# Vasilispapg/CVML-GoalNet

Measured on AMD Instinct MI355X. Metric: training clips/sec at batch 64, 16-frame 224² clips; logit MAE vs CPU ref, higher is better.
Workload: dtype f32; 1 GPU; AVM train step (forward + broadcast-MSE + backward + fused Adam), 64 clips x 16 frames = 1024 frames of 3x224x224 + 30x30 MFCC per GPU; dropout live (device masks), BatchNorm train mode; frames_per_gpu=1024, h=224, w=224, parallelism=dp1, ddp_semantics=local BN + local MSE per rank, gradient mean (standard DDP), params=1286754369

## Files before the change

### __graft_entry__.py

```python
from __future__ import annotations

import glob
import os
import subprocess
import sys

ROOT = os.path.dirname(os.path.abspath(__file__))
PKG = os.path.join(ROOT, "cvml_goalnet_amd")
CSRC = os.path.join(PKG, "csrc")
LIB = os.path.join(PKG, "libgoalnet_hip.so")
HIPCC = os.environ.get("HIPCC", "/opt/rocm/bin/hipcc")
FLAGS = ["--offload-arch=gfx950", "-O3", "-std=c++17", "-fPIC", "-Wall", "-Wno-unused-function"]


def _stale(target, sources):
    if not os.path.exists(target):
        return True
    t = os.path.getmtime(target)
    return any(os.path.getmtime(s) > t for s in sources)


def build(force: bool = False) -> None:
    srcs = sorted(glob.glob(os.path.join(CSRC, "*.hip")))
    hdrs = sorted(glob.glob(os.path.join(CSRC, "*.h"))) + [os.path.join(ROOT, "include", h) for h in ("goalnet_hip.h", "goalnet_loss.h")]
    objdir = os.path.join(CSRC, "build")
    os.makedirs(objdir, exist_ok=True)
    objs = []
    procs = []
    for s in srcs:
        o = os.path.join(objdir, os.path.basename(s)[:-4] + ".o")
        objs.append(o)
        if force or _stale(o, [s] + hdrs):
            procs.append((s, subprocess.Popen([HIPCC, *FLAGS, "-c", s, "-o", o])))
    for s, p in procs:
        if p.wait() != 0:
            raise RuntimeError(f"hipcc failed on {s}")
    if force or procs or _stale(LIB, objs):
        subprocess.check_call([HIPCC, "--offload-arch=gfx950", "-shared", "-fPIC", "-o", LIB, *objs])
    if ROOT not in sys.path:
        sys.path.insert(0, ROOT)
    import cvml_goalnet_amd
    from cvml_goalnet_amd import _lib
    lib = _lib.load()
    assert lib.goalnet_abi_version() == _lib.ABI_VERSION


def smoke() -> None:
    if ROOT not in sys.path:
        sys.path.insert(0, ROOT)
    import numpy as np
    import torch
    from cvml_goalnet_amd import AVM, synth
    from oracle import avm_ref

    assert torch.cuda.is_available(), "smoke() needs the GPU"
    torch.cuda.set_device(0)
    n, h = 4, 40
    params = synth.make_params(h, h)
    vis = torch.from_numpy(synth.make_visual(n, h, h))
    aud = torch.from_numpy(synth.make_audio(n))
    lab = torch.from_numpy(synth.make_labels(n))
    masks = [torch.from_numpy(m) for m in synth.make_drop_masks(n)]

    model = AVM(audio_included=True, device="cuda:0", seed=synth.BASE_SEED)
    sd = {k: torch.from_numpy(v) for k, v in params.items()}
    sd.update(avm_ref.init_buffers())
    model.load_state_dict(sd)
    loss, pred = model.train_step(aud.cuda(), vis.cuda(), lab.cuda())
    torch.cuda.synchronize()

    p = {k: torch.from_numpy(v.copy()) for k, v in params.items()}
    o_loss, o_pred, o_g = avm_ref.train_step(p, avm_ref.init_buffers(), {}, aud, vis, lab, masks, True)
    err = (pred.cpu() - o_pred.view(-1)).abs().max().item()
    lerr = abs(loss.item() - o_loss.item())
    new = model.state_dict()
    gerr = perr = 0.0
    for k, og in o_g.items():
# ... 16 lines not shown
```

### cvml_goalnet_amd/_lib.py

```python
from __future__ import annotations

import ctypes
import os
from ctypes import c_char_p, c_double, c_float, c_int, c_int64, c_size_t, c_uint32, c_uint64, c_void_p

_HERE = os.path.dirname(os.path.abspath(__file__))
LIB_PATH = os.environ.get("GOALNET_LIB_PATH") or os.path.join(_HERE, "libgoalnet_hip.so")
ABI_VERSION = 7
STAT_PARTS = 1024
ADAM_RANGES_MAX = 32

P = c_void_p


class RowCopy(ctypes.Structure):
    _fields_ = [("src", c_void_p), ("dst", c_void_p), ("row_bytes", c_int64), ("nrows", c_int), ("gather", c_int), ("cursor", c_void_p),
                ("cursor_bias", c_int64)]


class AdamRange(ctypes.Structure):
    _fields_ = [("begin", c_int64), ("count", c_int64), ("skipped", c_int64)]


PROTOTYPES = {
# ... 91 lines not shown
    "goalnet_mse_bcast": (c_int, [P, P, c_int, P, P, P]),
    "goalnet_cubic_resample": (c_int, [P, P, P, c_int64, c_int, c_int, P]),
    "goalnet_logmel_slots": (c_int, [P, P, P, c_int, c_int, P, P, P, P, P, P, P, P]),
    "goalnet_mfcc_from_logmel": (c_int, [P, P, c_int, c_int, P, P, P, P, c_int, c_int, c_double, P]),
    "goalnet_cls_head_fwd": (c_int, [P, c_int64, P, P, P, P, c_int, c_int, c_int, P]),
    "goalnet_cross_entropy": (c_int, [P, P, P, P, c_int, c_int, P]),
    "goalnet_cls_head_bwd": (c_int, [P, P, P, c_int64, P, P, c_int64, P, c_int64, P, P, c_int, c_int, c_int, P]),
    "goalnet_argmax_plus1": (c_int, [P, P, c_int, c_int, P]),
    "goalnet_adam_step": (c_int, [P, P, P, P, c_int64, c_double, c_double, c_double, c_double, c_int, c_float, P]),
    "goalnet_counter_add": (c_int, [P, c_int64, P]),
    "goalnet_dropout_masks_dev": (c_int, [P, c_int, ctypes.POINTER(c_int), c_int, c_uint64, c_uint32, c_uint32, P, c_float, c_int64, P]),
    "goalnet_adam_step_dev": (c_int, [P, P, P, P, c_int64, c_double, c_double, c_double, c_double, P, c_int64, c_float, P]),
    "goalnet_adam_step_dev_blocks": (c_int, [P, P, P, P, c_int64, c_double, c_double, c_double, c_double, P, c_int64, c_float, c_int, P]),
    "goalnet_adam_step_dev_shadow": (c_int, [P, P, P, P, c_int64, c_double, c_double, c_double, c_double, P, c_int64, c_float, P, c_int64,
                                             c_int64, c_int, P]),
    "goalnet_adam_step_dev_guarded": (c_int, [P, P, P, P, c_int64, c_double, c_double, c_double, c_double, P, c_int64, c_float, P, c_int64,
                                              c_int64, c_int, P, P]),
    "goalnet_adam_step_dev_ranges": (c_int, [P, P, P, P, ctypes.POINTER(AdamRange), c_int, c_double, c_double, c_double, c_double, P, c_float,
                                             P, c_int64, c_int64, c_int, P, P]),
    "goalnet_scale": (c_int, [P, c_int64, c_float, P]),
    "goalnet_grad_finite_check": (c_int, [P, c_int64, P, c_int64, P, P, P]),
    "goalnet_counters_add4": (c_int, [P, c_int64, c_int64, c_int64, c_int64, P]),
    "goalnet_counters_add4_guarded": (c_int, [P, c_int64, c_int64, c_int64, c_int64, P, P]),
    "goalnet_rows_scatter_tick": (c_int, [ctypes.POINTER(RowCopy), c_int, P, c_int64, c_int64, c_int64, c_int64, P, P]),
    "goalnet_rows_copy_batch": (c_int, [ctypes.POINTER(RowCopy), c_int, P]),
    "goalnet_frames_preprocess": (c_int, [P, c_int, c_int, c_int, P, c_int, c_int, P, P]),
    "goalnet_frames_preprocess_strided": (c_int, [P, c_int, c_int, c_int, c_int, P, c_int, c_int, P, P]),
    "goalnet_gather_clips_ws_bytes": (c_size_t, [c_int]),
    "goalnet_gather_clips": (c_int, [P, c_int, c_int64, P, P, c_int, P, c_int64, P, P, P, P, c_size_t, P]),
    "goalnet_kts_ws_bytes": (c_size_t, [c_int, c_int, c_int]),
    "goalnet_kts": (c_int, [P, c_int, c_int, c_int, c_int, c_int, c_int, c_double, c_int, c_int, P, P, P, P, P, P, P, c_size_t, P]),
    "goalnet_rank_corr": (c_int, [P, c_int64, c_int, P, c_int64, c_int, c_int, c_int, c_int, P, P, P, P, P, P, P]),
    "goalnet_knapsack_ws_bytes": (c_size_t, [c_int, c_int]),
    "goalnet_knapsack": (c_int, [P, P, c_int, c_int, P, P, c_size_t, P]),
    "goalnet_fscore": (c_int, [P, P, c_int, c_int, P, P, P]),
    "goalnet_postprocess_ws_bytes": (c_size_t, [c_int, c_int, c_int]),
    "goalnet_postprocess": (c_int, [P, c_int, c_int, c_int, P, c_int, c_int, c_int, P, c_int, P, P, P, P, P, P, P, c_size_t, P]),
    "goalnet_postprocess_batch_ws_bytes": (c_size_t, [c_int, c_int, c_int, c_int]),
    "goalnet_postprocess_batch": (c_int, [P, c_int, c_int, c_int, c_int, P, c_int, c_int, c_int, P, c_int, P, P, P, P, P, P, P, c_size_t, P]),
    "goalnet_postprocess_batch_kernel_name": (c_char_p, [c_int, c_int]),
    "goalnet_mean_annotations": (c_int, [P, c_int, c_int, c_int, P, P, P]),
    "goalnet_rows_gather": (c_int, [P, P, c_int64, c_int, P, P]),
    "goalnet_rows_scatter": (c_int, [P, P, c_int64, c_int, P, P]),
}

LOSS_PROTOTYPES = {
    "goalnet_frame_loss_ws_bytes": (c_size_t, [c_int, c_int]),
    "goalnet_frame_loss": (c_int, [c_int, c_double, P, P, P, c_int, P, P, P, c_size_t, P]),
    "goalnet_mlp_fwd_loss": (c_int, [P, c_int64, c_int, P, P, P, P, P, P, P, P, P, P, P, c_int, c_double, P, c_int, P, P]),
}
LOSS_KINDS = {"mse_bcast": 0, "mse": 1, "l1": 2, "smooth_l1": 3, "rank": 4}
FRAME_LOSS_MAX_N = 65536

_lib = None


class GoalnetError(RuntimeError):
    pass


def load():
    global _lib
    if _lib is not None:
        return _lib
    if not os.path.exists(LIB_PATH):
        raise GoalnetError(
            f"{LIB_PATH} not found: build it with `python -c 'import __graft_entry__ as g; g.build()'`. "
            "There is no CPU / eager fallback for the AVM hot path.")
    lib = ctypes.CDLL(LIB_PATH)
    for name, (res, args) in (*PROTOTYPES.items(), *LOSS_PROTOTYPES.items()):
        fn = getattr(lib, name)
        fn.restype = res
        fn.argtypes = args
    v = lib.goalnet_abi_version()
    if v != ABI_VERSION:
        raise GoalnetError(f"libgoalnet_hip.so ABI {v} != expected {ABI_VERSION}")
    _lib = lib
    return lib


def check(rc: int, what: str = ""):
    if rc != 0:
        msg = load().goalnet_last_error()
        raise GoalnetError(f"{what}: rc={rc}: {msg.decode() if msg else ''}")
```

### cvml_goalnet_amd/csrc/gemm_f32.hip

```cpp
#include <stdlib.h>

#include "adam.h"
#include "gemm_common.h"
#include "skinny.h"

using namespace goalnet;

namespace {

constexpr int BM = 128, BN = 128, BK = 32;
constexpr int LDR = 128;
constexpr int OP_FLOATS = BM * BK;

__device__ __forceinline__ int kc_off(int row, int chunk) { return row * BK + ((chunk ^ ((row >> 1) & 7)) << 2); }

__device__ __forceinline__ float4 f4zero() { return make_float4(0.f, 0.f, 0.f, 0.f); }
__device__ __forceinline__ float4 f4fma(float4 v, float4 s, float4 t) {
    return make_float4(fmaf(v.x, s.x, t.x), fmaf(v.y, s.y, t.y), fmaf(v.z, s.z, t.z), fmaf(v.w, s.w, t.w));
}

typedef unsigned int u32x4 __attribute__((ext_vector_type(4)));
constexpr unsigned OOB = 0xFFFFFF00u;

__device__ __forceinline__ float4 f4sel(bool v, float4 a) { return v ? a : f4zero(); }

__device__ __forceinline__ __amdgpu_buffer_rsrc_t make_rsrc(const void* base, uint32_t bytes) {
    return __builtin_amdgcn_make_buffer_rsrc(const_cast<void*>(base), 0, (int)bytes, 0x00020000);
}
__device__ __forceinline__ float4 bload(__amdgpu_buffer_rsrc_t r, unsigned voff, unsigned soff) {
    const u32x4 v = __builtin_amdgcn_raw_buffer_load_b128(r, (int)voff, (int)soff, 0);
    return make_float4(__uint_as_float(v.x), __uint_as_float(v.y), __uint_as_float(v.z), __uint_as_float(v.w));
}
__device__ __forceinline__ uint32_t clamp_u32(int64_t v) {
    return v <= 0 ? 0u : (v > 0xFFFFFF00ll ? 0xFFFFFF00u : (uint32_t)v);
}

template <bool AFFINE>
struct KCLoader {
    struct P {
        const float* x; int64_t ld; int rows;
        const float* scale; const float* shift; int bnC;
        int convC;
    };
    static constexpr bool KC = true;
    static constexpr bool STRIP = false;
    static constexpr bool ONE_STAGE = false;
    static constexpr int ONE_STAGE_BLOCKS = 3;
    __amdgpu_buffer_rsrc_t rx, rsc, rsh;
    unsigned voff[4], vaff;
    int bnC, convC;
    float4 sc, sh;
    __device__ KCLoader(const P& p, int row0, int tid) {
        const int nrows = p.rows - row0 < BM ? p.rows - row0 : BM;
        rx = make_rsrc(p.x + (int64_t)row0 * p.ld, clamp_u32((int64_t)nrows * p.ld * 4));
// ... 896 lines not shown
            a.x = fmaf(-shv.x, u, a.x); a.y = fmaf(-shv.y, u, a.y); a.z = fmaf(-shv.z, u, a.z); a.w = fmaf(-shv.w, u, a.w);
        }
        if (ok && g == 0) {
            float* o = ep.out + row * ep.ld + col;
            o[0] = epi_apply(ep, a.x, row, col);
            o[1] = epi_apply(ep, a.y, row, col + 1);
            o[2] = epi_apply(ep, a.z, row, col + 2);
            o[3] = epi_apply(ep, a.w, row, col + 3);
        }
    }
}

constexpr bool EPI_PAIR_DX = true;
static int epi_store_mode(const EpiP& ep, bool a_kc, bool b_kc) {
    const char* e = getenv("GOALNET_F32_EPI_STORE");
    if ((e && e[0] == '0') || !a_kc) return EPI_ST_GLOBAL;
    const bool slab = ep.slab_stride > 0;
    const int mode = slab ? EPI_RAW : ep.mode;
    const int64_t ld = (slab && ep.slabs) ? (int64_t)ep.cols : ep.ld;
    if (mode != EPI_RAW && mode != EPI_BIAS_RELU) return EPI_ST_GLOBAL;
    if (ep.rows <= 0 || ep.cols <= 0 || ld < ep.cols || (int64_t)BM * ld * 4 >= 0xFFFFFF00ll) return EPI_ST_GLOBAL;
    if (e && e[0] == '1') return EPI_ST_BUF;
    return (EPI_PAIR_DX && !b_kc && mode == EPI_RAW) ? EPI_ST_BUF_PAIR : EPI_ST_BUF;
}

template <class AL, class BL, bool N64 = false>
int launch_gemm(const char* name, const typename AL::P& ap, const typename BL::P& bp, const EpiP& ep,
                int64_t M, int64_t N, int ktiles, int nsplit, int m_fast, hipStream_t st) {
    const int64_t tiles_m = (M + BM - 1) / BM, tiles_n = (N + (N64 ? 64 : BN) - 1) / (N64 ? 64 : BN);
    GN_REQUIRE(tiles_m * tiles_n < (1ll << 31), GOALNET_E_SHAPE, "%s: too many tiles", name);
    GN_REQUIRE(nsplit >= 1 && nsplit <= 65535, GOALNET_E_SHAPE, "%s: bad split count %d", name, nsplit);
    const int kps = (ktiles + nsplit - 1) / nsplit;
    GN_REQUIRE(!ep.tile_ctr || (ktiles + kps - 1) / kps == nsplit, GOALNET_E_SHAPE, "%s: fused split-K needs every split non-empty", name);
    const bool xcd_local = nsplit >= 8 && tiles_m * tiles_n <= 256 && tiles_m * tiles_n * ((nsplit + 7) / 8 * 8) < (1ll << 31);
    dim3 grid((unsigned)(tiles_m * tiles_n), (unsigned)nsplit, 1);
    if (xcd_local) grid = dim3((unsigned)(tiles_m * tiles_n * ((nsplit + 7) / 8 * 8)), 1, 1);
    static const int force_stages = getenv("GOALNET_F32_STAGES") ? atoi(getenv("GOALNET_F32_STAGES")) : 0;
    const int epi_st = epi_store_mode(ep, AL::KC, BL::KC);
    const bool one_stage = AL::STRIP || force_stages == 1 || (force_stages != 2 && AL::ONE_STAGE);
    if (one_stage) {
        hipLaunchKernelGGL((gemm_f32_kernel<AL, BL, N64, 1>), grid, dim3(256), 0, st, ap, bp, ep, (int)tiles_m, (int)tiles_n,
                           (m_fast & 1) | (epi_st << 1), ktiles, kps, xcd_local ? nsplit : 0);
        GN_LAUNCH_CHECK(name);
        return 0;
    }
    if constexpr (!AL::STRIP) {
        hipLaunchKernelGGL((gemm_f32_kernel<AL, BL, N64>), grid, dim3(256), 0, st, ap, bp, ep, (int)tiles_m, (int)tiles_n,
                           (m_fast & 1) | (epi_st << 1), ktiles, kps, xcd_local ? nsplit : 0);
        GN_LAUNCH_CHECK(name);
    }
    return 0;
}

}

namespace goalnet {
int launch_splitk_reduce(const char* name, const float* slabs, int nsplit, int64_t slab_stride, const EpiP& ep, hipStream_t st) {
    const int64_t total = (int64_t)ep.rows * (ep.cols >> 2);
    int64_t blocks = (total + 255) / 256;
    if (blocks > 4096) blocks = 4096;
    if (blocks < 1) blocks = 1;
    if (total < 65536 && nsplit >= 32) {
        int64_t wb = (total + 15) / 16;
        if (wb > 4096) wb = 4096;
        hipLaunchKernelGGL(splitk_reduce_wide_kernel, dim3((unsigned)wb), dim3(256), 0, st, slabs, nsplit, slab_stride, ep);
        GN_LAUNCH_CHECK(name);
        return 0;
    }
    hipLaunchKernelGGL(splitk_reduce_kernel, dim3((unsigned)blocks), dim3(256), 0, st, slabs, nsplit, slab_stride, ep);
    GN_LAUNCH_CHECK(name);
    return 0;
}

int pick_splits(int64_t tiles, int ktiles) {
    if (ktiles < 8 || (ktiles < 64 && tiles >= 128)) return 1;
    int64_t s = ((ktiles < 64 ? 256 : 1024) + tiles - 1) / tiles;
    const int64_t smax = ktiles < 64 ? ktiles / 4 : (ktiles / 8 > 1 ? ktiles / 8 : 1);
    if (s > smax) s = smax;
    if (s < 1) s = 1;
    const int kps = (int)((ktiles + s - 1) / s);
    return (ktiles + kps - 1) / kps;
}

}

extern "C" {

static int conv_splits_f32(int64_t M, int Cin, int Cout) {
    return conv_fwd_splits(((M + BM - 1) / BM) * ((Cout + BN - 1) / BN), 9 * Cin / BK);
}

constexpr bool CONV_STRIP_FWD = true;
constexpr bool CONV_STRIP_DGRAD = true;
static bool conv_strip_f32(int W, int nsplit, bool narrow, bool affine) {
    const char* e = getenv("GOALNET_F32_CONV_STRIP");
    if (e && e[0] == '0') return false;
    return nsplit == 1 && !narrow && W <= CONV_STRIP_MAX_W && (affine ? CONV_STRIP_FWD : CONV_STRIP_DGRAD);
}

size_t goalnet_conv3x3_fwd_ws_bytes(int N, int H, int W, int Cin, int Cout) {
    if (N <= 0 || H <= 0 || W <= 0 || Cin <= 0 || Cout <= 0) return 0;
    const int64_t M = (int64_t)N * H * W;
    const int s = conv_splits_f32(M, Cin, Cout);
    return s > 1 ? (size_t)s * (size_t)M * (size_t)Cout * sizeof(float) : 0;
}

// ... 45 lines not shown
    }
    if (rc || nsplit == 1 || fused) return rc;
    return launch_splitk_reduce("conv3x3_fwd.reduce", (const float*)ws, nsplit, M * Cout, efinal, st);
}

}
namespace {
template <class AL, class BL, bool N64, int STAGES> const char* gemm_f32_kernel_name_() { return __PRETTY_FUNCTION__; }
template <class AL, class BL, bool N64> const char* gemm_f32_kernel_name() {
    const int force = getenv("GOALNET_F32_STAGES") ? atoi(getenv("GOALNET_F32_STAGES")) : 0;
    const bool one = AL::STRIP || force == 1 || (force != 2 && AL::ONE_STAGE);
    return one ? gemm_f32_kernel_name_<AL, BL, N64, 1>() : gemm_f32_kernel_name_<AL, BL, N64, 2>();
}
}
extern "C" {

const char* goalnet_conv3x3_fwd_kernel_name(int N, int H, int W, int Cin, int Cout, int affine) {
    const bool narrow = Cout <= 64 && !getenv("GOALNET_F32_N64_OFF");
    const int nsplit = (N > 0 && H > 0 && W > 0 && Cin > 0 && Cout > 0) ? conv_splits_f32((int64_t)N * H * W, Cin, Cout) : 1;
    if (conv_strip_f32(W, nsplit, narrow, affine != 0))
        return affine ? gemm_f32_kernel_name<ConvAStripLoader<true>, KCLoader<false>, false>()
                      : gemm_f32_kernel_name<ConvAStripLoader<false>, KCLoader<false>, false>();
    if (affine) return narrow ? gemm_f32_kernel_name<ConvALoader<true>, KCLoader<false>, true>() : gemm_f32_kernel_name<ConvALoader<true>, KCLoader<false>, false>();
    return narrow ? gemm_f32_kernel_name<ConvALoader<false>, KCLoader<false>, true>() : gemm_f32_kernel_name<ConvALoader<false>, KCLoader<false>, false>();
}

static int wgrad_splits(int64_t M, int Cin, int Cout) {
    const int64_t tiles = (int64_t)((Cout + BM - 1) / BM) * ((9 * Cin + BN - 1) / BN);
    const int ktiles = (int)((M + BK - 1) / BK);
    static const int wtarget = getenv("GOALNET_WGRAD_SPLIT_TARGET") ? atoi(getenv("GOALNET_WGRAD_SPLIT_TARGET")) : 2048;
    int64_t s = (wtarget + tiles - 1) / tiles;
    const int64_t smax = ktiles / 4 > 1 ? ktiles / 4 : 1;
    if (s > smax) s = smax;
    if (s > 512) s = 512;
    if (s >= 8) {
        int64_t best = (s + 7) / 8 * 8 <= smax ? (s + 7) / 8 * 8 : s / 8 * 8;
        double best_eff = 0.0;
        for (int64_t c = best; c <= 2 * s + 8 && c <= smax && c <= 1024; c += 8) {
            const int64_t blocks = tiles * c, rounds = (blocks + 511) / 512;
            const double eff = (double)blocks / (double)(rounds * 512);
            if (eff > best_eff + 1e-9) { best_eff = eff; best = c; }
        }
        s = best;
    }
    const int kps = (int)((ktiles + s - 1) / s);
    return (ktiles + kps - 1) / kps;
}

static size_t wgrad_codes_bytes(int64_t M) { return (size_t)((M + 31) / 32 * 32 + 255) / 256 * 256; }
static size_t wgrad_border_bytes(int N, int Cout) {
    return ((size_t)N * 8 * Cout * sizeof(double) + 255) / 256 * 256 + ((size_t)Cout * 9 * sizeof(float) + 255) / 256 * 256;
}

size_t goalnet_conv3x3_wgrad_ws_bytes(int N, int H, int W, int Cin, int Cout) {
    const int64_t M = (int64_t)N * H * W;
    return wgrad_codes_bytes(M) + wgrad_border_bytes(N, Cout) + (size_t)wgrad_splits(M, Cin, Cout) * (size_t)Cout * 9 * Cin * sizeof(float);
}

int goalnet_conv3x3_wgrad_codes(uint32_t* codes, int N, int H, int W, void* stream) {
    GN_REQUIRE(codes && N > 0 && H > 0 && W > 0, GOALNET_E_NULL, "conv3x3_wgrad_codes: bad arguments");
    const int64_t M = (int64_t)N * H * W;
    GN_REQUIRE(M < (1ll << 31) - 256, GOALNET_E_SHAPE, "conv3x3_wgrad_codes: N*H*W too large");
    const int Mpad = (int)((M + 31) / 32 * 32);
    int blocks = (Mpad / 4 + 255) / 256;
    if (blocks > 4096) blocks = 4096;
    hipLaunchKernelGGL(border_codes_kernel, dim3(blocks), dim3(256), 0, (hipStream_t)stream, codes, (int)M, Mpad, H, W);
    GN_LAUNCH_CHECK("conv3x3_wgrad_codes");
    return 0;
}

size_t goalnet_conv3x3_wgrad_codes_bytes(int N, int H, int W) { return wgrad_codes_bytes((int64_t)N * H * W); }

int goalnet_conv3x3_wgrad(const float* x, const float* scale, const float* shift, const float* dy, float* dw,
                          void* ws, size_t ws_bytes, const uint32_t* codes_in, int* tile_ctr, int n_ctr,
                          int N, int H, int W, int Cin, int Cout, void* stream) {
    GN_REQUIRE(x && dy && dw && ws, GOALNET_E_NULL, "conv3x3_wgrad: null pointer");
    GN_REQUIRE((scale == nullptr) == (shift == nullptr), GOALNET_E_NULL, "conv3x3_wgrad: scale/shift must both be set or both NULL");
    GN_REQUIRE(N > 0 && H > 0 && W > 0, GOALNET_E_SHAPE, "conv3x3_wgrad: non-positive dim");
    GN_REQUIRE(Cin % 4 == 0 && Cout % 4 == 0 && Cin > 0 && Cout > 0, GOALNET_E_SHAPE, "conv3x3_wgrad: channels must be multiples of 4");
    GN_REQUIRE(aligned16(x) && aligned16(dy) && aligned16(dw) && aligned16(ws) && aligned16(scale) && aligned16(shift),
               GOALNET_E_ALIGN, "conv3x3_wgrad: pointers must be 16-byte aligned");
    const int64_t M = (int64_t)N * H * W;
    GN_REQUIRE(M < (1ll << 31) - 256, GOALNET_E_SHAPE, "conv3x3_wgrad: N*H*W too large");
    GN_REQUIRE(ws_bytes >= goalnet_conv3x3_wgrad_ws_bytes(N, H, W, Cin, Cout), GOALNET_E_WORKSPACE, "conv3x3_wgrad: workspace too small");
    hipStream_t st = (hipStream_t)stream;
    const int nsplit = wgrad_splits(M, Cin, Cout);
    const int ktiles = (int)((M + BK - 1) / BK);
    const int64_t slab = (int64_t)Cout * 9 * Cin;
    uint32_t* codes = (uint32_t*)ws;
    double* bparts = (double*)((char*)ws + wgrad_codes_bytes(M));
    float* bu = (float*)((char*)bparts + ((size_t)N * 8 * Cout * sizeof(double) + 255) / 256 * 256);
    float* slabs = (float*)((char*)ws + wgrad_codes_bytes(M) + wgrad_border_bytes(N, Cout));
    const char* force = getenv("GOALNET_WGRAD_PATH");
    const bool dsel = force && force[0] == 's' ? true : force && force[0] == 'c' ? false : (int64_t)N * (H > W ? H : W) <= 4096;
    if (codes_in) {
        codes = const_cast<uint32_t*>(codes_in);
    } else {
        const int Mpad = (int)((M + 31) / 32 * 32);
        int blocks = (Mpad / 4 + 255) / 256;
        if (blocks > 4096) blocks = 4096;
        hipLaunchKernelGGL(border_codes_kernel, dim3(blocks), dim3(256), 0, st, codes, (int)M, Mpad, H, W);
        GN_LAUNCH_CHECK("conv3x3_wgrad.codes");
    }
    if (scale && !dsel) {
        hipLaunchKernelGGL(wgrad_border_sums_kernel, dim3(N), dim3(256), 0, st, dy, bparts, H, W, Cout);
        GN_LAUNCH_CHECK("conv3x3_wgrad.border_sums");
        hipLaunchKernelGGL(wgrad_border_u_kernel, dim3((Cout + 31) / 32), dim3(256), 0, st, bparts, N, Cout, bu);
        GN_LAUNCH_CHECK("conv3x3_wgrad.border_u");
    }
    MCLoader<false>::P ap{dy, Cout, Cout, (int)M, nullptr, nullptr, 1};
    EpiP ep{EPI_RAW, slabs, (int64_t)9 * Cin, Cout, 9 * Cin, nullptr, 0, nullptr, 0, nullptr, 0, slab};
    const bool fused = nsplit > 1 && tile_ctr && (dsel || !scale) &&
                       (int64_t)n_ctr >= (int64_t)((Cout + BM - 1) / BM) * ((9 * Cin + BN - 1) / BN);
    if (fused) {
        ep = EpiP{EPI_RAW, dw, (int64_t)9 * Cin, Cout, 9 * Cin, nullptr, 0, nullptr, 0, nullptr, 0, slab};
        ep.slabs = slabs; ep.tile_ctr = tile_ctr;
    }
    int rc;
    if (scale && dsel) {
        ConvWgradBLoader<true, true>::P bp{x, H, W, Cin, (int)M, scale, shift, codes};
        rc = launch_gemm<MCLoader<false>, ConvWgradBLoader<true, true>>("conv3x3_wgrad", ap, bp, ep, Cout, 9 * Cin, ktiles, nsplit, 1, st);
    } else if (scale) {
        ConvWgradBLoader<true>::P bp{x, H, W, Cin, (int)M, scale, shift, codes};
        rc = launch_gemm<MCLoader<false>, ConvWgradBLoader<true>>("conv3x3_wgrad", ap, bp, ep, Cout, 9 * Cin, ktiles, nsplit, 1, st);
    } else {
        ConvWgradBLoader<false>::P bp{x, H, W, Cin, (int)M, nullptr, nullptr, codes};
        rc = launch_gemm<MCLoader<false>, ConvWgradBLoader<false>>("conv3x3_wgrad", ap, bp, ep, Cout, 9 * Cin, ktiles, nsplit, 1, st);
    }
    if (rc || fused) return rc;
    EpiP er{EPI_RAW, dw, (int64_t)9 * Cin, Cout, 9 * Cin, nullptr, 0, nullptr, 0, nullptr, 0, 0};
    if (scale && !dsel) { er.corr_u = bu; er.corr_sh = shift; er.corr_C = Cin; }
    return launch_splitk_reduce("conv3x3_wgrad.reduce", slabs, nsplit, slab, er, st);
}

static int linear_splits(int M, int64_t K, int J) {
    const int64_t tiles = (int64_t)((M + BM - 1) / BM) * ((J + BN - 1) / BN);
    return pick_splits(tiles, (int)(K / BK));
}

size_t goalnet_linear_fwd_ws_bytes(int M, int64_t K, int J) {
    if (M <= 0 || K <= 0 || J <= 0) return 0;
    if (M <= SKINNY_MAX_M) return skinny_fwd_ws_bytes(M, K, J);
    const int s = linear_splits(M, K, J);
    return s > 1 ? (size_t)s * (size_t)M * (size_t)J * sizeof(float) : 0;
}

int goalnet_linear_fwd(const float* x, int64_t ldx, const float* scale, const float* shift, int bnC,
// ... 109 lines not shown
```

Before: 161.8 clips/s.

## Add strip-based MFMA conv3x3 weight-gradient kernel reusing LDS input strip across taps

Adds a new f32 conv3x3 weight-gradient path. It stages a contiguous strip of input rows (with halo) in LDS once per chunk and computes all nine taps from it with hand-scheduled inline-asm MFMA 32x32x2 instructions. Border taps are masked using ballot-derived masks instead of precomputed border codes, and the BN affine is applied while staging. Partial results go through split-K slabs and a reduce kernel, replacing the codes and border-sum kernels for large-batch shapes. This is meant to cut redundant input loads and im2col-style overhead. In exchange it adds heavy inline asm with hard-coded AGPR clobbers and a new split heuristic that could enlarge the workspace.

New measurement: 163.2 clips/s, median of 6. No clear change (+0.8%).

```diff
diff --git a/__graft_entry__.py b/__graft_entry__.py
--- a/__graft_entry__.py
+++ b/__graft_entry__.py
@@ -22,7 +22,7 @@
 
 def build(force: bool = False) -> None:
     srcs = sorted(glob.glob(os.path.join(CSRC, "*.hip")))
-    hdrs = sorted(glob.glob(os.path.join(CSRC, "*.h"))) + [os.path.join(ROOT, "include", h) for h in ("goalnet_hip.h", "goalnet_loss.h")]
+    hdrs = sorted(glob.glob(os.path.join(CSRC, "*.h"))) + [os.path.join(ROOT, "include", h) for h in ("goalnet_hip.h", "goalnet_loss.h", "goalnet_wgrad.h")]
     objdir = os.path.join(CSRC, "build")
     os.makedirs(objdir, exist_ok=True)
     objs = []
diff --git a/cvml_goalnet_amd/_lib.py b/cvml_goalnet_amd/_lib.py
--- a/cvml_goalnet_amd/_lib.py
+++ b/cvml_goalnet_amd/_lib.py
@@ -167,6 +167,12 @@
 LOSS_KINDS = {"mse_bcast": 0, "mse": 1, "l1": 2, "smooth_l1": 3, "rank": 4}
 FRAME_LOSS_MAX_N = 65536
 
+WGRAD_PROTOTYPES = {
+    "goalnet_conv3x3_wgrad_path": (c_int, [c_int, c_int, c_int, c_int, c_int, c_int, c_int]),
+    "goalnet_conv3x3_wgrad_strip_max_w": (c_int, []),
+    "goalnet_conv3x3_wgrad_path_splits": (c_int, [c_int, c_int, c_int, c_int, c_int, c_int]),
+}
+
 _lib = None
 
 
@@ -183,7 +189,7 @@
             f"{LIB_PATH} not found: build it with `python -c 'import __graft_entry__ as g; g.build()'`. "
             "There is no CPU / eager fallback for the AVM hot path.")
     lib = ctypes.CDLL(LIB_PATH)
-    for name, (res, args) in (*PROTOTYPES.items(), *LOSS_PROTOTYPES.items()):
+    for name, (res, args) in (*PROTOTYPES.items(), *LOSS_PROTOTYPES.items(), *WGRAD_PROTOTYPES.items()):
         fn = getattr(lib, name)
         fn.restype = res
         fn.argtypes = args
diff --git a/cvml_goalnet_amd/csrc/gemm_f32.hip b/cvml_goalnet_amd/csrc/gemm_f32.hip
--- a/cvml_goalnet_amd/csrc/gemm_f32.hip
+++ b/cvml_goalnet_amd/csrc/gemm_f32.hip
@@ -1,5 +1,6 @@
 #include <stdlib.h>
 
+#include "../../include/goalnet_wgrad.h"
 #include "adam.h"
 #include "gemm_common.h"
 #include "skinny.h"
@@ -1002,6 +1003,303 @@
     return 0;
 }
 
+constexpr int WS_CI = 32;
+constexpr int WS_CHUNK = 4 * BK;
+constexpr int WGRAD_STRIP_MAX_W = CONV_STRIP_MAX_W;
+
+struct WgradStripP {
+    const float* x; const float* dy; const float* scale; const float* shift;
+    float* slabs; int64_t slab_stride;
+    int H, W, Cin, Cout, M;
+    int nchunks, chunks_per_split, nsplit, tiles_m, tiles_n;
+};
+
+__device__ __forceinline__ float zero_where(float a, uint64_t m) {
+    float o;
+    asm volatile("v_cndmask_b32_e64 %0, %1, 0, %2" : "=v"(o) : "v"(a), "s"(m));
+    return o;
+}
+__device__ __forceinline__ uint64_t step_mask(uint32_t m, int kk) {
+    const uint32_t lo = (uint32_t)((int32_t)(m << (31 - kk)) >> 31);
+    const uint32_t hi = (uint32_t)((int32_t)(m << (27 - kk)) >> 31);
+    return ((uint64_t)hi << 32) | lo;
+}
+
+typedef __attribute__((address_space(3))) const float lds_cfloat;
+__device__ __forceinline__ unsigned lds_addr(const float* p) { return (unsigned)(uintptr_t)(lds_cfloat*)p; }
+template <int OFF>
+__device__ __forceinline__ void ws_ds_read(float& d, unsigned addr) {
+    static_assert(OFF >= 0 && OFF < 65536, "16-bit immediate");
+    asm volatile("ds_read_b32 %0, %1 offset:%2" : "=v"(d) : "v"(addr), "n"(OFF));
+}
+__device__ __forceinline__ void ws_wait(float& a, float (&b)[9]) {
+    asm volatile("s_waitcnt lgkmcnt(0)"
+                 : "+v"(a), "+v"(b[0]), "+v"(b[1]), "+v"(b[2]), "+v"(b[3]), "+v"(b[4]), "+v"(b[5]), "+v"(b[6]), "+v"(b[7]), "+v"(b[8]));
+}
+#define WS_CL10(d) "a" #d "0", "a" #d "1", "a" #d "2", "a" #d "3", "a" #d "4", "a" #d "5", "a" #d "6", "a" #d "7", "a" #d "8", "a" #d "9"
+#define WS_ACC_CLOBBERS                                                                                                          \
+    "a0", "a1", "a2", "a3", "a4", "a5", "a6", "a7", "a8", "a9", WS_CL10(1), WS_CL10(2), WS_CL10(3), WS_CL10(4), WS_CL10(5),       \
+        WS_CL10(6), WS_CL10(7), WS_CL10(8), WS_CL10(9), WS_CL10(10), WS_CL10(11), WS_CL10(12), WS_CL10(13), "a140", "a141", "a142", \
+        "a143"
+#define WS_A0 "a[0:15]"
+#define WS_A1 "a[16:31]"
+#define WS_A2 "a[32:47]"
+#define WS_A3 "a[48:63]"
+#define WS_A4 "a[64:79]"
+#define WS_A5 "a[80:95]"
+#define WS_A6 "a[96:111]"
+#define WS_A7 "a[112:127]"
+#define WS_A8 "a[128:143]"
+#define WS_TAP(ACC, T) "v_mfma_f32_32x32x2_f32 " ACC ", %[v" #T "], %[b" #T "], " ACC "\n\t"
+#define WS_TAP_RD(ACC, T) WS_TAP(ACC, T) "ds_read_b32 %[b" #T "], %[t" #T "] offset:%[ob]\n\t"
+#define WS_STEP_OPERANDS                                                                                                          \
+    [b0] "+v"(b[0]), [b1] "+v"(b[1]), [b2] "+v"(b[2]), [b3] "+v"(b[3]), [b4] "+v"(b[4]), [b5] "+v"(b[5]), [b6] "+v"(b[6]),         \
+        [b7] "+v"(b[7]), [b8] "+v"(b[8])                                                                                          \
+        : [v0] "v"(av[0]), [v1] "v"(av[1]), [v2] "v"(av[2]), [v3] "v"(av[3]), [v4] "v"(av[4]), [v5] "v"(av[5]), [v6] "v"(av[6]),   \
+          [v7] "v"(av[7]), [v8] "v"(av[8]), [t0] "v"(tb[0]), [t1] "v"(tb[1]), [t2] "v"(tb[2]), [t3] "v"(tb[3]), [t4] "v"(tb[4]),   \
+          [t5] "v"(tb[5]), [t6] "v"(tb[6]), [t7] "v"(tb[7]), [t8] "v"(tb[8]), [ob] "n"(OB)                                         \
+        : WS_ACC_CLOBBERS
+template <int OB, bool NEXT>
+__device__ __forceinline__ void ws_mfma9(const float (&av)[9], float (&b)[9], const unsigned (&tb)[9]) {
+    if constexpr (NEXT)
+        asm volatile(WS_TAP_RD(WS_A4, 4) WS_TAP_RD(WS_A1, 1) WS_TAP_RD(WS_A7, 7) WS_TAP_RD(WS_A0, 0) WS_TAP_RD(WS_A3, 3)
+                         WS_TAP_RD(WS_A6, 6) WS_TAP_RD(WS_A2, 2) WS_TAP_RD(WS_A5, 5) WS_TAP_RD(WS_A8, 8)
+                     : WS_STEP_OPERANDS);
+    else
+        asm volatile(WS_TAP(WS_A4, 4) WS_TAP(WS_A1, 1) WS_TAP(WS_A7, 7) WS_TAP(WS_A0, 0) WS_TAP(WS_A3, 3) WS_TAP(WS_A6, 6)
+                         WS_TAP(WS_A2, 2) WS_TAP(WS_A5, 5) WS_TAP(WS_A8, 8)
+                     : WS_STEP_OPERANDS);
+}
+__device__ __forceinline__ void ws_acc_zero() {
+    const float z = 0.f;
+#define WS_Z(ACC) "v_mfma_f32_32x32x2_f32 " ACC ", %0, %0, 0\n\t"
+    asm volatile(WS_Z(WS_A0) WS_Z(WS_A1) WS_Z(WS_A2) WS_Z(WS_A3) WS_Z(WS_A4) WS_Z(WS_A5) WS_Z(WS_A6) WS_Z(WS_A7) WS_Z(WS_A8)
+                 :
+                 : "v"(z)
+                 : WS_ACC_CLOBBERS);
+#undef WS_Z
+}
+__device__ __forceinline__ void ws_acc_settle() { asm volatile("s_nop 15\n\ts_nop 15" ::: "memory"); }
+template <int T>
+__device__ __forceinline__ f32x16 ws_acc_get() {
+    f32x16 v;
+    if constexpr (T == 0) asm volatile("" : "={a[0:15]}"(v));
+    if constexpr (T == 1) asm volatile("" : "={a[16:31]}"(v));
+    if constexpr (T == 2) asm volatile("" : "={a[32:47]}"(v));
+    if constexpr (T == 3) asm volatile("" : "={a[48:63]}"(v));
+    if constexpr (T == 4) asm volatile("" : "={a[64:79]}"(v));
+    if constexpr (T == 5) asm volatile("" : "={a[80:95]}"(v));
+    if constexpr (T == 6) asm volatile("" : "={a[96:111]}"(v));
+    if constexpr (T == 7) asm volatile("" : "={a[112:127]}"(v));
+    if constexpr (T == 8) asm volatile("" : "={a[128:143]}"(v));
+    return v;
+}
+template <bool FULL, int T>
+__device__ __forceinline__ void ws_store_tap(__amdgpu_buffer_rsrc_t rs, unsigned vo, unsigned ld4, int C, int rl0, int nrows) {
+    const f32x16 v = ws_acc_get<T>();
+#pragma unroll
+    for (int e = 0; e < 16; ++e)
+        bstore<FULL>(rs, v[e], vo, (unsigned)((e & 3) + 8 * (e >> 2)) * ld4 + (unsigned)(T * C) * 4u, rl0 + (e & 3) + 8 * (e >> 2), nrows);
+}
+template <bool FULL>
+__device__ __forceinline__ void ws_store_all(__amdgpu_buffer_rsrc_t rs, unsigned vo, unsigned ld4, int C, int rl0, int nrows) {
+    ws_store_tap<FULL, 0>(rs, vo, ld4, C, rl0, nrows); ws_store_tap<FULL, 1>(rs, vo, ld4, C, rl0, nrows);
+    ws_store_tap<FULL, 2>(rs, vo, ld4, C, rl0, nrows); ws_store_tap<FULL, 3>(rs, vo, ld4, C, rl0, nrows);
+    ws_store_tap<FULL, 4>(rs, vo, ld4, C, rl0, nrows); ws_store_tap<FULL, 5>(rs, vo, ld4, C, rl0, nrows);
+    ws_store_tap<FULL, 6>(rs, vo, ld4, C, rl0, nrows); ws_store_tap<FULL, 7>(rs, vo, ld4, C, rl0, nrows);
+    ws_store_tap<FULL, 8>(rs, vo, ld4, C, rl0, nrows);
+}
+
+template <int MODE, int Q, int ST>
+struct WgradStripSteps {
+    static __device__ __forceinline__ void run(unsigned pa, const unsigned (&tb)[9], const uint32_t (&cw)[2], const uint32_t (&ch)[2],
+                                               float a, float (&b)[9]) {
+        constexpr int kk = 8 * (ST >> 2) + (ST & 3);
+        constexpr int kkn = 8 * ((ST + 1) >> 2) + ((ST + 1) & 3);
+        ws_wait(a, b);
+        float av[9];
+#pragma unroll
+        for (int t = 0; t < 9; ++t) av[t] = a;
+        if constexpr (MODE == 1) {
+            av[0] = av[3] = av[6] = zero_where(a, step_mask(cw[0], kk));
+            av[2] = av[5] = av[8] = zero_where(a, step_mask(cw[1], kk));
+        } else if constexpr (MODE == 2) {
+            const uint64_t mw[3] = {step_mask(cw[0], kk), 0ull, step_mask(cw[1], kk)};
+            const uint64_t mh[3] = {step_mask(ch[0], kk), 0ull, step_mask(ch[1], kk)};
+#pragma unroll
+            for (int t = 0; t < 9; ++t)
+                if (t != 4) av[t] = zero_where(a, mh[t / 3] | mw[t % 3]);
+        }
+        float an = 0.f;
+        if constexpr (ST < 15) ws_ds_read<(Q & 1) * OP_FLOATS * 4 + kkn * LDR * 4>(an, pa);
+        ws_mfma9<(Q * BK + kkn) * WS_CI * 4, (ST < 15)>(av, b, tb);
+        if constexpr (ST < 15) WgradStripSteps<MODE, Q, ST + 1>::run(pa, tb, cw, ch, an, b);
+    }
+};
+
+template <int MODE, int Q>
+__device__ __forceinline__ void wgrad_strip_tile(unsigned pa, const unsigned (&tb)[9], const uint32_t (&cw)[2], const uint32_t (&ch)[2]) {
+    float a, b[9];
+    ws_ds_read<(Q & 1) * OP_FLOATS * 4>(a, pa);
+#pragma unroll
+    for (int t = 0; t < 9; ++t) ws_ds_read<Q * BK * WS_CI * 4>(b[t], tb[t]);
+    WgradStripSteps<MODE, Q, 0>::run(pa, tb, cw, ch, a, b);
+}
+
+template <int Q>
+__device__ __forceinline__ void wgrad_strip_tile_any(unsigned pa, const unsigned (&tb)[9],
+                                                     const uint64_t (&bw)[2][2], const uint64_t (&bh)[2][2]) {
+    const uint32_t cw[2] = {(uint32_t)(bw[0][Q >> 1] >> (32 * (Q & 1))), (uint32_t)(bw[1][Q >> 1] >> (32 * (Q & 1)))};
+    const uint32_t ch[2] = {(uint32_t)(bh[0][Q >> 1] >> (32 * (Q & 1))), (uint32_t)(bh[1][Q >> 1] >> (32 * (Q & 1)))};
+    if ((ch[0] | ch[1]) != 0) wgrad_strip_tile<2, Q>(pa, tb, cw, ch);
+    else if ((cw[0] | cw[1]) != 0) wgrad_strip_tile<1, Q>(pa, tb, cw, ch);
+    else wgrad_strip_tile<0, Q>(pa, tb, cw, ch);
+}
+
+__device__ __forceinline__ float4 wgrad_strip_load(const float* x, int C, int ci0, int W, int M, int c, int i, unsigned voff, int rr) {
+    const int64_t lo = (int64_t)c * WS_CHUNK - (W + 1) + 32 * i;
+    const int rows_left = WS_CHUNK + 2 * (W + 1) - 32 * i;
+    const int64_t hi = lo + (rows_left < 32 ? (rows_left < 0 ? 0 : rows_left) : 32);
+    const int64_t n = (hi < M ? hi : (int64_t)M) - lo;
+    const __amdgpu_buffer_rsrc_t rx = make_rsrc(x + lo * C + ci0, n > 0 ? (uint32_t)(((n - 1) * C + WS_CI) * 4) : 0u);
+    if (lo < 0) return bload(rx, lo + rr < 0 ? OOB : voff, 0);
+    return bload(rx, voff, 0);
+}
+
+template <bool AFFINE>
+__device__ __forceinline__ void wgrad_strip_store(float* ls, const float4 (&rs)[STRIP_LOADS], const float* laff, int tid) {
+    const int c4 = (tid & 7) * 4, rr = tid >> 3;
+    float4 sc = f4zero(), sh = f4zero();
+    if (AFFINE) {
+        sc = *reinterpret_cast<const float4*>(&laff[c4]);
+        sh = *reinterpret_cast<const float4*>(&laff[WS_CI + c4]);
+    }
+#pragma unroll
+    for (int i = 0; i < STRIP_LOADS; ++i)
+        *reinterpret_cast<float4*>(&ls[(rr + 32 * i) * WS_CI + c4]) = AFFINE ? f4fma(rs[i], sc, sh) : rs[i];
+}
+
+__device__ __forceinline__ void wgrad_strip_advance(int& h, int& w, int dh, int dw, int H, int W) {
+    w += dw;
+    const bool carry = w >= W;
+    w -= carry ? W : 0;
+    h += dh + (carry ? 1 : 0);
+    h -= h >= H ? H : 0;
+}
+
+template <bool AFFINE>
+__global__ __launch_bounds__(256, 1) void wgrad_strip_kernel(WgradStripP p) {
+    const int tid = threadIdx.x;
+    const int tiles = p.tiles_m * p.tiles_n;
+    const int xcd = blockIdx.x & 7, bj = blockIdx.x >> 3;
+    const int grp = bj / tiles, t = bj - grp * tiles;
+    const int split = grp * 8 + xcd;
+    if (split >= p.nsplit) return;
+    const int tm = t % p.tiles_m, tn = t / p.tiles_m;
+    const int c0 = split * p.chunks_per_split;
+    const int c1 = min(p.nchunks, c0 + p.chunks_per_split);
+    const int ci0 = tn * WS_CI;
+    const int H = p.H, W = p.W, C = p.Cin, M = p.M;
+    const int lane = tid & 63, wave = tid >> 6;
+    const int r = lane & 31, h = lane >> 5;
+
+    __shared__ __attribute__((aligned(16))) float lstrip[STRIP_ROWS * WS_CI];
+    __shared__ __attribute__((aligned(16))) float ldy[2][OP_FLOATS];
+
+    MCLoader<false>::P ap{p.dy, p.Cout, p.Cout, M, nullptr, nullptr, 1};
+    MCLoader<false> al(ap, tm * BM, tid);
+
+    ws_acc_zero();
+
+    const int rr = tid >> 3;
+    const unsigned voff = (unsigned)((rr * C + (tid & 7) * 4) * 4);
+    __shared__ __attribute__((aligned(16))) float laff[2 * WS_CI];
+    if (AFFINE) {
+        if (tid < 8) *reinterpret_cast<float4*>(&laff[tid * 4]) = *reinterpret_cast<const float4*>(p.scale + ci0 + tid * 4);
+        else if (tid < 16) *reinterpret_cast<float4*>(&laff[tid * 4]) = *reinterpret_cast<const float4*>(p.shift + ci0 + (tid - 8) * 4);
+        __syncthreads();
+    }
+    const unsigned pa = lds_addr(&ldy[0][0]) + (unsigned)((4 * h * LDR + 32 * wave + r) * 4);
+    unsigned tb[9];
+#pragma unroll
+    for (int q = 0; q < 9; ++q) tb[q] = lds_addr(lstrip) + (unsigned)(((4 * h + (q / 3) * W + (q % 3)) * WS_CI + r) * 4);
+    int ph[2], pw[2];
+#pragma unroll
+    for (int q = 0; q < 2; ++q) {
+        const unsigned m = (unsigned)c0 * WS_CHUNK + (unsigned)(64 * q + lane);
+        pw[q] = (int)(m % (unsigned)W);
+        ph[q] = (int)((m / (unsigned)W) % (unsigned)H);
+    }
+    const int dw = WS_CHUNK % W, dh = (WS_CHUNK / W) % H;
+
+    float4 rs[STRIP_LOADS], ra[4];
+    if (c0 < c1) {
+#pragma unroll
+        for (int i = 0; i < STRIP_LOADS; ++i) rs[i] = wgrad_strip_load(p.x, C, ci0, W, M, c0, i, voff, rr);
+        al.issue(c0 * 4, ra);
+        wgrad_strip_store<AFFINE>(lstrip, rs, laff, tid);
+        store_tile<false>(ldy[0], ra, tid);
+    }
+    __syncthreads();
+    for (int c = c0; c < c1; ++c) {
+        const bool next = c + 1 < c1;
+        uint64_t bw[2][2], bh[2][2];
+#pragma unroll
+        for (int q = 0; q < 2; ++q) {
+            bw[0][q] = __builtin_amdgcn_ballot_w64(pw[q] == 0);
+            bw[1][q] = __builtin_amdgcn_ballot_w64(pw[q] == W - 1);
+            bh[0][q] = __builtin_amdgcn_ballot_w64(ph[q] == 0);
+            bh[1][q] = __builtin_amdgcn_ballot_w64(ph[q] == H - 1);
+            wgrad_strip_advance(ph[q], pw[q], dh, dw, H, W);
+        }
+        al.issue(c * 4 + 1, ra);
+        if (next) {
+#pragma unroll
+            for (int i = 0; i < 3; ++i) rs[i] = wgrad_strip_load(p.x, C, ci0, W, M, c + 1, i, voff, rr);
+        }
+        wgrad_strip_tile_any<0>(pa, tb, bw, bh);
+        store_tile<false>(ldy[1], ra, tid);
+        __syncthreads();
+        al.issue(c * 4 + 2, ra);
+        if (next) {
+#pragma unroll
+            for (int i = 3; i < 5; ++i) rs[i] = wgrad_strip_load(p.x, C, ci0, W, M, c + 1, i, voff, rr);
+        }
+        wgrad_strip_tile_any<1>(pa, tb, bw, bh);
+        store_tile<false>(ldy[0], ra, tid);
+        __syncthreads();
+        al.issue(c * 4 + 3, ra);
+        if (next) {
+#pragma unroll
+            for (int i = 5; i < 7; ++i) rs[i] = wgrad_strip_load(p.x, C, ci0, W, M, c + 1, i, voff, rr);
+        }
+        wgrad_strip_tile_any<2>(pa, tb, bw, bh);
+        store_tile<false>(ldy[1], ra, tid);
+        __syncthreads();
+        if (next) {
+            al.issue(c * 4 + 4, ra);
+#pragma unroll
+            for (int i = 7; i < 9; ++i) rs[i] = wgrad_strip_load(p.x, C, ci0, W, M, c + 1, i, voff, rr);
+        }
+        wgrad_strip_tile_any<3>(pa, tb, bw, bh);
+        if (next) {
+            store_tile<false>(ldy[0], ra, tid);
+            __syncthreads();
+            wgrad_strip_store<AFFINE>(lstrip, rs, laff, tid);
+        }
+        __syncthreads();
+    }
+
+    ws_acc_settle();
+    const int nrows = p.Cout - tm * BM < BM ? p.Cout - tm * BM : BM;
+    const unsigned ld4 = (unsigned)(9 * C) * 4u;
+    const __amdgpu_buffer_rsrc_t rs_out = make_rsrc(p.slabs + (int64_t)split * p.slab_stride + (int64_t)tm * BM * 9 * C, (uint32_t)nrows * ld4);
+    const int rl0 = 32 * wave + 4 * h;
+    const unsigned vo = (unsigned)rl0 * ld4 + (unsigned)(ci0 + r) * 4u;
+    if (nrows == BM) ws_store_all<true>(rs_out, vo, ld4, C, rl0, nrows);
+    else ws_store_all<false>(rs_out, vo, ld4, C, rl0, nrows);
+}
+
 }
 
 namespace goalnet {
@@ -1153,9 +1451,58 @@
     return ((size_t)N * 8 * Cout * sizeof(double) + 255) / 256 * 256 + ((size_t)Cout * 9 * sizeof(float) + 255) / 256 * 256;
 }
 
+static int wgrad_strip_splits(int64_t M, int Cin, int Cout) {
+    const int64_t tiles = (int64_t)((Cout + BM - 1) / BM) * (Cin / WS_CI);
+    const int64_t nchunks = M > 0 ? (M + WS_CHUNK - 1) / WS_CHUNK : 1;
+    int64_t s = (512 + (tiles > 0 ? tiles : 1) - 1) / (tiles > 0 ? tiles : 1);
+    const int64_t smax = nchunks / 2 > 1 ? nchunks / 2 : 1;
+    if (s > smax) s = smax;
+    if (s > 512) s = 512;
+    if (s >= 8) {
+        int64_t best = (s + 7) / 8 * 8 <= smax ? (s + 7) / 8 * 8 : s / 8 * 8;
+        double best_eff = 0.0;
+        for (int64_t c = best; c <= 2 * s + 8 && c <= smax && c <= 1024; c += 8) {
+            const int64_t blocks = tiles * c, rounds = (blocks + 511) / 512;
+            const double eff = (double)blocks / (double)(rounds * 512);
+            if (eff > best_eff + 1e-9) { best_eff = eff; best = c; }
+        }
+        s = best;
+    }
+    const int64_t cps = (nchunks + s - 1) / s;
+    return (int)((nchunks + cps - 1) / cps);
+}
+
+constexpr bool WGRAD_STRIP_ADOPTED = true;
+static bool wgrad_dsel(int N, int H, int W) {
+    const char* force = getenv("GOALNET_WGRAD_PATH");
+    return force && force[0] == 's' ? true : force && force[0] == 'c' ? false : (int64_t)N * (H > W ? H : W) <= 4096;
+}
+static bool wgrad_strip_f32(int N, int H, int W, int Cin, bool affine, bool has_ctr) {
+    const char* e = getenv("GOALNET_F32_WGRAD_STRIP");
+    if (e && e[0] == '0') return false;
+    const bool dsel = wgrad_dsel(N, H, W);
+    const bool legal = Cin % WS_CI == 0 && W <= WGRAD_STRIP_MAX_W && !(has_ctr && (dsel || !affine));
+    if (e && e[0] == '1') return legal;
+    return legal && !dsel && WGRAD_STRIP_ADOPTED;
+}
+
+int goalnet_conv3x3_wgrad_path(int N, int H, int W, int Cin, int Cout, int affine, int has_ctr) {
+    if (N <= 0 || H <= 0 || W <= 0 || Cin <= 0 || Cout <= 0) return -1;
+    return wgrad_strip_f32(N, H, W, Cin, affine != 0, has_ctr != 0) ? 1 : 0;
+}
+
+int goalnet_conv3x3_wgrad_strip_max_w(void) { return WGRAD_STRIP_MAX_W; }
+
+int goalnet_conv3x3_wgrad_path_splits(int N, int H, int W, int Cin, int Cout, int strip) {
+    const int64_t M = (int64_t)N * H * W;
+    return strip ? (Cin % WS_CI == 0 ? wgrad_strip_splits(M, Cin, Cout) : 0) : wgrad_splits(M, Cin, Cout);
+}
+
 size_t goalnet_conv3x3_wgrad_ws_bytes(int N, int H, int W, int Cin, int Cout) {
     const int64_t M = (int64_t)N * H * W;
-    return wgrad_codes_bytes(M) + wgrad_border_bytes(N, Cout) + (size_t)wgrad_splits(M, Cin, Cout) * (size_t)Cout * 9 * Cin * sizeof(float);
+    int s = wgrad_splits(M, Cin, Cout);
+    if (Cin > 0 && Cin % WS_CI == 0 && W <= WGRAD_STRIP_MAX_W) { const int t = wgrad_strip_splits(M, Cin, Cout); s = t > s ? t : s; }
+    return wgrad_codes_bytes(M) + wgrad_border_bytes(N, Cout) + (size_t)s * (size_t)Cout * 9 * Cin * sizeof(float);
 }
 
 int goalnet_conv3x3_wgrad_codes(uint32_t* codes, int N, int H, int W, void* stream) {
@@ -1192,8 +1539,21 @@
     double* bparts = (double*)((char*)ws + wgrad_codes_bytes(M));
     float* bu = (float*)((char*)bparts + ((size_t)N * 8 * Cout * sizeof(double) + 255) / 256 * 256);
     float* slabs = (float*)((char*)ws + wgrad_codes_bytes(M) + wgrad_border_bytes(N, Cout));
-    const char* force = getenv("GOALNET_WGRAD_PATH");
-    const bool dsel = force && force[0] == 's' ? true : force && force[0] == 'c' ? false : (int64_t)N * (H > W ? H : W) <= 4096;
+    const bool dsel = wgrad_dsel(N, H, W);
+    if (wgrad_strip_f32(N, H, W, Cin, scale != nullptr, tile_ctr != nullptr)) {
+        const int ssplit = wgrad_strip_splits(M, Cin, Cout);
+        const int nchunks = (int)((M + WS_CHUNK - 1) / WS_CHUNK);
+        const int tiles_m = (Cout + BM - 1) / BM, tiles_n = Cin / WS_CI;
+        GN_REQUIRE((int64_t)tiles_m * tiles_n * ((ssplit + 7) / 8 * 8) < (1ll << 31), GOALNET_E_SHAPE, "conv3x3_wgrad: too many tiles");
+        const WgradStripP sp{x, dy, scale, shift, slabs, slab, H, W, Cin, Cout, (int)M, nchunks, (nchunks + ssplit - 1) / ssplit, ssplit,
+                             tiles_m, tiles_n};
+        const dim3 grid((unsigned)(tiles_m * tiles_n * ((ssplit + 7) / 8 * 8)), 1, 1);
+        if (scale) hipLaunchKernelGGL(wgrad_strip_kernel<true>, grid, dim3(256), 0, st, sp);
+        else hipLaunchKernelGGL(wgrad_strip_kernel<false>, grid, dim3(256), 0, st, sp);
+        GN_LAUNCH_CHECK("conv3x3_wgrad.strip");
+        const EpiP er{EPI_RAW, dw, (int64_t)9 * Cin, Cout, 9 * Cin, nullptr, 0, nullptr, 0, nullptr, 0, 0};
+        return launch_splitk_reduce("conv3x3_wgrad.reduce", slabs, ssplit, slab, er, st);
+    }
     if (codes_in) {
         codes = const_cast<uint32_t*>(codes_in);
     } else {
diff --git a/include/goalnet_wgrad.h b/include/goalnet_wgrad.h
--- /dev/null
+++ b/include/goalnet_wgrad.h
@@ -0,0 +1,20 @@
+#ifndef GOALNET_WGRAD_H
+#define GOALNET_WGRAD_H
+
+#include "goalnet_hip.h"
+
+#ifdef __cplusplus
+extern "C" {
+#endif
+
+int goalnet_conv3x3_wgrad_path(int N, int H, int W, int Cin, int Cout, int affine, int has_ctr);
+
+int goalnet_conv3x3_wgrad_strip_max_w(void);
+
+int goalnet_conv3x3_wgrad_path_splits(int N, int H, int W, int Cin, int Cout, int strip);
+
+#ifdef __cplusplus
+}
+#endif
+
+#endif
```
